# PAMRec/PAMRec

Measured on NVIDIA B200. Metric: train samples/sec, higher is better.
Workload: dtype f32

## Files before the change

### pamrec_b200/csrc/api.cu

```cuda
#include <cmath>
#include <cstdarg>
#include <cstdio>
#include <cstdlib>
#include <string>
#include <vector>

#include "comm.h"
#include "head2.h"
#include "kernels.h"
#include "layout.h"

using namespace pamrec;

struct Xchg {
  std::vector<int64_t> soff, scnt, roff, rcnt;
  int64_t n_send = 0, n_recv = 0;
};

struct PamrecHandle_ {
  PamrecConfig cfg;
  Layout L;
  PamrecBuffers buf;
  bool bound = false;
  int debug = 0;
  std::string err;
  int64_t launches = 0;
  Prof prof;
  BnSet bn[BN_COUNT];
  std::vector<int> h_seg_id, h_seg_tab;
  Comm comm;
  int* h_counts = nullptr;
  Xchg xc[3];
  bool xc_users = false;
  bool sharded() const { return cfg.table_mode == PAMREC_TABLES_SHARDED; }
  bool sibling() const { return cfg.model_kind != PAMREC_MODEL_PAMREC; }
  bool replicated() const { return cfg.table_mode == PAMREC_TABLES_REPLICATED && cfg.world_size > 1; }
  cudaStream_t side = nullptr;
  cudaEvent_t ev_side[12] = {};
  cudaEvent_t ev_join = nullptr, ev_plan = nullptr, ev_bucket = nullptr;
  int ev_next = 0;
  const void* plan_for = nullptr;
  int plan_rows = -1;
  void* mbox = nullptr;
  void* mbox_peer[kP2PMaxWorld] = {};
  bool mbox_open = false;
  unsigned* head_bar = nullptr;
  bool head_trace = false;
  unsigned long long* head_trace_cta = nullptr;
  uint32_t coop_epoch = 0;
  Head2 head2;
  int head2_grid = 0;
  bool use_head2() const { return head2_grid > 0 && (cfg.world_size == 1 || mbox_open); }
  uint32_t* mbox_err() const { return static_cast<uint32_t*>(mbox); }
  int64_t xr_dense() const { return (L.dense_numel + 63) / 64 * 64; }
  int64_t xr_floats() const { return xr_dense() + (replicated() ? sp2_rep_floats(cfg.n_items, cfg.n_cates, cfg.n_users) : 0); }
  char* xr_region(int p) const { return static_cast<char*>(mbox_peer[p]) + p2p_xr_offset(cfg.world_size); }
  bool use_xr() const { return mbox_open && cfg.world_size > 1; }
  uint32_t xr_epoch = 0;
  float* rep_grad_in() const { return use_xr() ? xr_xbuf(xr_region(cfg.rank)) + xr_dense() : wf("rep.grad"); }
  float* rep_grad_out() const {
    return use_xr() ? xr_xbuf(xr_region(cfg.rank)) + p2p_xr_cap(cfg.world_size, xr_floats()) + xr_dense() : wf("rep.grad");
  }
  ~PamrecHandle_() {
    if (h_counts) cudaFreeHost(h_counts);
    for (int p = 0; p < kP2PMaxWorld; ++p)
      if (mbox_peer[p] && mbox_peer[p] != mbox) cudaIpcCloseMemHandle(mbox_peer[p]);
    if (mbox) cudaFree(mbox);
    if (head_bar) cudaFree(head_bar);
    if (head_trace_cta) cudaFree(head_trace_cta);
    for (auto e : ev_side) if (e) cudaEventDestroy(e);
    if (ev_join) cudaEventDestroy(ev_join);
    if (ev_plan) cudaEventDestroy(ev_plan);
    if (ev_bucket) cudaEventDestroy(ev_bucket);
    if (side) cudaStreamDestroy(side);
  }
  template <typename F>
  void fork(cudaStream_t main, F fn) {
    cudaEvent_t e = ev_side[ev_next];
    ev_next = (ev_next + 1) % 12;
    cudaEventRecord(e, main);
    cudaStreamWaitEvent(side, e, 0);
    fn(side);
  }
  void join(cudaStream_t main) {
    cudaEventRecord(ev_join, side);
    cudaStreamWaitEvent(main, ev_join, 0);
  }

  float* P(int64_t off) const { return buf.dense_param + off; }
  float* G(int64_t off) const { return buf.dense_grad + off; }
  template <typename T>
  T* ws(const std::string& name) const { return reinterpret_cast<T*>(static_cast<char*>(buf.workspace) + L.ws_off(name)); }
  float* wf(const std::string& name) const { return ws<float>(name); }
  int* wi(const std::string& name) const { return ws<int>(name); }
  double* wd(const std::string& name) const { return ws<double>(name); }
};

struct ProfBind {
  PamrecHandle h; int64_t l0; Prof* prev;
  explicit ProfBind(PamrecHandle hh) : h(hh), l0(hh->prof.launches), prev(g_prof) { g_prof = &hh->prof; }
  ~ProfBind() { h->launches = h->prof.launches - l0; g_prof = prev; }
};
// ... 798 lines not shown
  const int B = b->batch, T = h->cfg.max_seq_len, N = B * T;
  int crc = 0;
  cudaMemsetAsync(h->buf.dense_grad, 0, (size_t)L.dense_numel * 4, st);
  cudaMemsetAsync(h->wd("loss_acc"), 0, 8 * sizeof(double), st);
  cudaMemsetAsync(h->wd("sp_normsq"), 0, 8 * sizeof(double), st);
  if (h->use_head2()) {
    cudaMemsetAsync(h->wd("bn.bsums"), 0, (size_t)L.ws[L.ws_index.at("bn.bsums")].numel * sizeof(double), st);
    HeadDyn d = head_dyn(h, b, true, 12);
    if (launch_head2_bwd(h->head2, d, h->head2_grid, st)) return check_cuda(h, "cooperative head launch");
    h->fork(st, [&](cudaStream_t s2) { launch_head2_dw(h->head2, B, s2); });
  } else {
    crc = head_backward(h, b, st);
  }
  float* g_a = h->wf("g_a");
  float* g_b = h->wf("g_b");
  const int max_tiles = N / kTokTile + kNB + 1;
  int* ctl = h->wi("bucket_ctl");
  for (int k = 1; k >= 0; --k) {
    const BlockOff& o = L.blk[k];
    std::string p = "blk" + std::to_string(k) + ".";
    const float* xin = k == 0 ? h->wf("x0") : h->wf("blk0.out");
    float* gout = k == 1 ? g_a : g_b;
    float* gin = k == 1 ? g_b : g_a;
    launch_ffn_bwd(h->wf(p + "y"), gout, h->P(o.w1), h->P(o.b1), h->P(o.w2), h->P(o.ln_b_beta), h->P(o.ln_b_gamma), h->wf("d_y"),
                   h->G(o.w1), h->G(o.b1), h->G(o.w2), h->G(o.b2), h->G(o.ln_b_beta), h->G(o.ln_b_gamma), N, st);
    if (T <= 128)
      launch_attn_bwd_mma(h->wf(p + "Q"), h->wf(p + "K"), h->wf(p + "V"), h->wf("d_y"), h->wf(p + "pv"), h->wf(p + "ml"),
                          b->mask, h->wf("d_Q"), h->wf("d_K"), h->wf("d_V"), B, T, st);
    else
      launch_attn_bwd(h->wf(p + "Q"), h->wf(p + "K"), h->wf(p + "V"), h->wf("d_y"), h->wf(p + "pv"), h->wf(p + "ml"),
                      b->mask, h->wf("d_Q"), h->wf("d_K"), h->wf("d_V"), B, T, st);
    launch_proj_bwd(xin, h->wf("d_y"), h->wf("d_Q"), h->wf("d_K"), h->wf("d_V"), h->wi("perm"), ctl, h->wi("tile_bucket"),
                    h->wi("tile_begin"), h->wi("tile_count"), max_tiles, h->P(o.wq), h->P(o.wk), h->P(o.wv), h->P(o.ln_a_beta),
                    h->P(o.ln_a_gamma), gin, h->G(o.wq), h->G(o.wk), h->G(o.wv), h->G(o.ln_a_beta), h->G(o.ln_a_gamma), st);
  }
  launch_embed_bwd_reduce(g_a, h->wf("d_tgt"), h->wf("d_tgt_total"), h->G(L.pos), h->wd("sp_normsq") + 4,
                          h->sharded() ? nullptr : h->wd("sp_normsq"), B, T, st);
  h->join(st);
  if (crc) return fail(h, "nccl: %s", h->comm.err.c_str());
  return check_cuda(h, "backward");
}

static void peer_allreduce_grads(PamrecHandle h, cudaStream_t st) {
  XrArgs a;
  memset(&a, 0, sizeof a);
  const int W = h->cfg.world_size;
  for (int p = 0; p < W; ++p) a.peer[p] = h->xr_region(p);
  a.world = W; a.rank = h->cfg.rank; a.epoch = ++h->xr_epoch;
  a.cap = p2p_xr_cap(W, h->xr_floats());
  a.dense_grad = h->buf.dense_grad; a.n_dense = h->L.dense_numel;
  a.scalars[0] = h->wd("sp_normsq"); a.n_scalars[0] = 8;
  a.scalars[1] = h->wd("loss_acc"); a.n_scalars[1] = 4;
  a.counter = reinterpret_cast<unsigned*>(h->xr_region(h->cfg.rank) + 128);
  a.err = h->mbox_err();
  launch_xr_allreduce(a, h->buf.dense_grad, st);
}

// ... 230 lines not shown
```

### pamrec_b200/csrc/kernels.h

```cpp
#pragma once
#include <string>
#include <vector>

#include "common.cuh"

namespace pamrec {

struct Prof {
  bool on = false;
  int64_t launches = 0;
  std::vector<std::string> names;
  std::vector<double> ms;
  std::vector<int64_t> cnt;
  struct Pair { cudaEvent_t a, b; int id; };
  std::vector<Pair> pending;
  std::vector<cudaEvent_t> free_ev;
  int id_of(const char* name);
  cudaEvent_t get_event();
  void resolve();
  void reset();
  ~Prof();
};
extern thread_local Prof* g_prof;
struct ProfScope {
  Prof* p; cudaStream_t st; cudaEvent_t b; bool timed;
  ProfScope(const char* name, int n_kernels, cudaStream_t st);
  ~ProfScope();
};
#define PAMREC_PROF(name, n, st) ProfScope _prof_scope(name, n, st)

int init_encoder_kernels(int max_T);
void launch_embed_fwd(const int* ih, const int* ch, const int* items, const int* cates, const float* item_w,
                      const float* cate_w, const float* pos, float* x0, float* tgt, int64_t n_rows, int T, cudaStream_t st);
void launch_bucket_plan(const float* lt, int n, int* bucket, int* perm, int* ctl, int* tile_bucket, int* tile_begin,
                        int* tile_count, cudaStream_t st);
void launch_proj_fwd(const float* X, const int* perm, const int* ctl, const int* tile_bucket, const int* tile_begin,
                     const int* tile_count, int max_tiles, const float* Wq, const float* Wk, const float* Wv,
                     const float* ln_beta, const float* ln_gamma, float* QIN, float* Q, float* K, float* V, cudaStream_t st);
void launch_attn_fwd(const float* Q, const float* K, const float* V, const float* QIN, const int* mask, float* Y, float* PV,
                     float* ML, int B, int T, cudaStream_t st);
void launch_ffn_fwd(const float* Y, const float* W1, const float* b1, const float* W2, const float* b2,
                    const float* ln_beta, const float* ln_gamma, float* OUT, float* Hdbg, int n_tok, cudaStream_t st);
void launch_ffn_bwd(const float* Y, const float* dOUT, const float* W1, const float* b1, const float* W2,
                    const float* ln_beta, const float* ln_gamma, float* dY, float* dW1, float* db1, float* dW2,
                    float* db2, float* dbeta, float* dgamma, int n_tok, cudaStream_t st);
void launch_attn_bwd(const float* Q, const float* K, const float* V, const float* dY, const float* PV, const float* ML,
                     const int* mask, float* dQ, float* dK, float* dV, int B, int T, cudaStream_t st);
void launch_proj_bwd(const float* X, const float* dY, const float* dQ, const float* dK, const float* dV, const int* perm,
                     const int* ctl, const int* tile_bucket, const int* tile_begin, const int* tile_count, int max_tiles,
                     const float* Wq, const float* Wk, const float* Wv, const float* ln_beta, const float* ln_gamma,
                     float* dX, float* dWq, float* dWk, float* dWv, float* dbeta, float* dgamma, cudaStream_t st);

int init_attn_mma_kernels(int max_T);
void launch_attn_fwd_mma(const float* Q, const float* K, const float* V, const float* QIN, const int* mask, float* Y, float* PV, float* ML,
                         int B, int T, cudaStream_t st);
void launch_attn_bwd_mma(const float* Q, const float* K, const float* V, const float* dY, const float* PV, const float* ML,
                         const int* mask, float* dQ, float* dK, float* dV, int B, int T, cudaStream_t st);

void launch_dense_fwd(const DenseP& p, cudaStream_t st);
void launch_dense_dx(const DenseDxP& p, cudaStream_t st);
void launch_dense_dw(const DenseDwP& p, cudaStream_t st);
void launch_bn_finalize(const BnSet& s, double count, cudaStream_t st);
void launch_bn_eval_stat(const BnSet& s, cudaStream_t st);
void launch_bn_bwd_stats(const BnSet& s, const float* dA, const float* Z, int M, cudaStream_t st);
void launch_pool_fwd(const float* H, const float* Z2, const BnSet& s1, const int* mask, float* new_long, int B, int T,
                     cudaStream_t st);
void launch_pool_bwd(const float* H, const float* Z2, const BnSet& s1, const int* mask, const float* d_new_long, float* dA2,
                     float* dH, int B, int T, cudaStream_t st);
void launch_combine_fwd(const float* ZE1, const float* ZG1, const BnSet& e1, const BnSet& g1, const float* tgt, float* U,
                        int B, cudaStream_t st);
void launch_combine_bwd(const float* ZE1, const float* ZG1, const BnSet& e1, const BnSet& g1, const float* dU, float* dE1,
                        float* dG1, float* dTgt, int B, cudaStream_t st);
void launch_loss(const float* logits, const float* y_sat, const float* y_play, const float* plays, float* d_logits,
                 double* loss_acc, int B, int B_global, const double* n_valid_global, float fuzhu_w, float order_w,
// ... 132 lines not shown
```

### pamrec_b200/csrc/kernels_encoder.cu

```cuda
#include "kernels.h"
#include "mma.cuh"

namespace pamrec {

constexpr int kEmbU = 8;
constexpr int kEmbTok = 32;
__global__ void __launch_bounds__(kEmbTok * 10, 3)
k_embed_fwd(const int* __restrict__ ih, const int* __restrict__ ch, const int* __restrict__ items,
            const int* __restrict__ cates, const float* __restrict__ item_w, const float* __restrict__ cate_w,
            const float* __restrict__ pos, float* __restrict__ x0, float* __restrict__ tgt, int64_t n_tok, int T) {
  constexpr int TOK = kEmbTok * kEmbU;
  __shared__ int s_id[4][TOK];
  __shared__ int s_t[TOK];
  const int tid = threadIdx.x;
  const int64_t tok0 = (int64_t)blockIdx.x * TOK;
  for (int i = tid; i < TOK; i += kEmbTok * 10) {
    const int64_t tok = tok0 + i;
    if (tok < n_tok) {
      const int64_t b = tok / T;
      s_t[i] = (int)(tok - b * T);
      s_id[0][i] = __ldg(ih + tok);
      s_id[1][i] = __ldg(ch + tok);
      s_id[2][i] = __ldg(items + b);
      s_id[3][i] = __ldg(cates + b);
// ... 487 lines not shown
    for (int j = 0; j < 2; ++j) {
      float a = sb[nt][j], b = sg[nt][j];
#pragma unroll
      for (int o = 4; o < 32; o <<= 1) { a += __shfl_xor_sync(0xffffffffu, a, o); b += __shfl_xor_sync(0xffffffffu, b, o); }
      if (g == 0) { atomicAdd(red + 8 * nt + 2 * t + j, a); atomicAdd(red + kD + 8 * nt + 2 * t + j, b); }
    }
}
__device__ __forceinline__ void store_frag_rows(float* __restrict__ dst, const float (&c)[kMT][5][4], int64_t tok0, const int* toks,
                                                int row_base, int cnt, int lane) {
  const int g = lane >> 2, t = lane & 3;
#pragma unroll
  for (int mt = 0; mt < kMT; ++mt)
#pragma unroll
    for (int h = 0; h < 2; ++h) {
      const int r = row_base + 16 * mt + g + 8 * h;
      if (r < cnt) {
        float* o = dst + (toks ? (int64_t)toks[r] : tok0 + r) * kD + 2 * t;
#pragma unroll
        for (int nt = 0; nt < 5; ++nt) *reinterpret_cast<float2*>(o + 8 * nt) = make_float2(c[mt][nt][2 * h], c[mt][nt][2 * h + 1]);
      }
    }
}

constexpr int kFfnBwdSmem = (4 * kDD + 3 * kTokTile * kTS + 2 * 41 * kD + 4 * kD + 2 * kD + kTokTile) * 4;
__global__ void __launch_bounds__(kTokThreads)
k_ffn_bwd(const float* __restrict__ Y, const float* __restrict__ dOUT, const float* __restrict__ W1,
          const float* __restrict__ b1, const float* __restrict__ W2, const float* __restrict__ ln_beta,
          const float* __restrict__ ln_gamma, float* __restrict__ dY, float* __restrict__ dW1, float* __restrict__ db1,
          float* __restrict__ dW2, float* __restrict__ db2, float* __restrict__ dbeta, float* __restrict__ dgamma,
          int n_tok) {
  extern __shared__ __align__(16) float sm[];
  uint32_t* W1hi = reinterpret_cast<uint32_t*>(sm);
  uint32_t* W1lo = W1hi + kDD;
  uint32_t* W2hi = W1lo + kDD;
  uint32_t* W2lo = W2hi + kDD;
  float* xs = sm + 4 * kDD;
  float* hs = xs + kTokTile * kTS;
  float* gs = hs + kTokTile * kTS;
  float* acc2 = gs + kTokTile * kTS;
  float* acc1 = acc2 + 41 * kD;
  float* pr = acc1 + 41 * kD;
  float* red = pr + 4 * kD;
  float* rstd_s = red + 2 * kD;
  const int tid = threadIdx.x, lane = tid & 31, w = tid >> 5;
  const int g = lane >> 2, t = lane & 3;
  const int64_t tok0 = (int64_t)blockIdx.x * kTokTile;
  const int cnt = (int)min((int64_t)kTokTile, (int64_t)n_tok - tok0);
  load_split_mat(W1hi, W1lo, W1, tid);
  load_split_mat(W2hi, W2lo, W2, tid);
  if (tid < kD) { pr[tid] = b1[tid]; pr[2 * kD + tid] = ln_beta[tid]; pr[3 * kD + tid] = ln_gamma[tid]; }
  if (tid < 2 * kD) red[tid] = 0.f;
  for (int i = tid; i < 2 * 41 * kD; i += kTokThreads) acc2[i] = 0.f;
  load_tile44(xs, Y + tok0 * kD, nullptr, cnt, tid);
  load_tile44(gs, dOUT + tok0 * kD, nullptr, cnt, tid);
  __syncthreads();
  if (tid < kTokTile) {
    float mean, rstd;
    ln_row44(xs + tid * kTS, pr + 2 * kD, pr + 3 * kD, mean, rstd, kLnWriteXhat);
    rstd_s[tid] = rstd;
  }
  __syncthreads();
  const float* xw = xs + kWarpRows * w * kTS;
  float* hw = hs + kWarpRows * w * kTS;
  const float* gw = gs + kWarpRows * w * kTS;
  const float* beta = pr + 2 * kD;
  const float* gamma = pr + 3 * kD;
  auto f_elem = [&](int r, int k) { return fmaf(gamma[k], xw[r * kTS + k], beta[k]); };
  float c[kMT][5][4];
#pragma unroll
  for (int mt = 0; mt < kMT; ++mt)
#pragma unroll
    for (int nt = 0; nt < 5; ++nt) {
      const float b0 = pr[8 * nt + 2 * t], bb1 = pr[8 * nt + 2 * t + 1];
      c[mt][nt][0] = b0; c[mt][nt][1] = bb1; c[mt][nt][2] = b0; c[mt][nt][3] = bb1;
    }
  warp_gemm_rows_x40x40<kMT, false>(c, f_elem, W1hi, W1lo, lane);
#pragma unroll
  for (int mt = 0; mt < kMT; ++mt)
#pragma unroll
    for (int nt = 0; nt < 5; ++nt) {
      const int r = 16 * mt + g, col = 8 * nt + 2 * t;
      *reinterpret_cast<float2*>(hw + r * kTS + col) = make_float2(fmaxf(c[mt][nt][0], 0.f), fmaxf(c[mt][nt][1], 0.f));
      *reinterpret_cast<float2*>(hw + (r + 8) * kTS + col) = make_float2(fmaxf(c[mt][nt][2], 0.f), fmaxf(c[mt][nt][3], 0.f));
    }
  __syncwarp();
#pragma unroll
  for (int mt = 0; mt < kMT; ++mt)
#pragma unroll
    for (int nt = 0; nt < 5; ++nt)
#pragma unroll
      for (int q = 0; q < 4; ++q) c[mt][nt][q] = 0.f;
  warp_gemm_rows_x40x40<kMT, true>(c, [&](int r, int k) { return gw[r * kTS + k]; }, W2hi, W2lo, lane);
#pragma unroll
  for (int mt = 0; mt < kMT; ++mt)
#pragma unroll
    for (int nt = 0; nt < 5; ++nt) {
      const int r = 16 * mt + g, col = 8 * nt + 2 * t;
      const float2 h0 = *reinterpret_cast<const float2*>(hw + r * kTS + col);
      const float2 h1 = *reinterpret_cast<const float2*>(hw + (r + 8) * kTS + col);
      if (!(h0.x > 0.f)) c[mt][nt][0] = 0.f;
      if (!(h0.y > 0.f)) c[mt][nt][1] = 0.f;
      if (!(h1.x > 0.f)) c[mt][nt][2] = 0.f;
      if (!(h1.y > 0.f)) c[mt][nt][3] = 0.f;
    }
  {
    float cw[3][5][4];
#pragma unroll
    for (int mt = 0; mt < 3; ++mt)
#pragma unroll
      for (int nt = 0; nt < 5; ++nt)
#pragma unroll
        for (int q = 0; q < 4; ++q) cw[mt][nt][q] = 0.f;
    warp_gemm_tn_48x40(cw, kWarpRows, [&](int r, int i) { return i < kD ? hw[r * kTS + i] : (i == kD ? 1.f : 0.f); },
                       [&](int r, int n) { return gw[r * kTS + n]; }, lane);
    tn_flush_smem(cw, acc2, lane);
  }
  __syncwarp();
#pragma unroll
  for (int mt = 0; mt < kMT; ++mt)
#pragma unroll
    for (int nt = 0; nt < 5; ++nt) {
      const int r = 16 * mt + g, col = 8 * nt + 2 * t;
      *reinterpret_cast<float2*>(hw + r * kTS + col) = make_float2(c[mt][nt][0], c[mt][nt][1]);
      *reinterpret_cast<float2*>(hw + (r + 8) * kTS + col) = make_float2(c[mt][nt][2], c[mt][nt][3]);
    }
  __syncwarp();
#pragma unroll
  for (int mt = 0; mt < kMT; ++mt)
#pragma unroll
    for (int nt = 0; nt < 5; ++nt) {
      const int r = 16 * mt + g, col = 8 * nt + 2 * t;
      const float2 g0 = *reinterpret_cast<const float2*>(gw + r * kTS + col);
      const float2 g1 = *reinterpret_cast<const float2*>(gw + (r + 8) * kTS + col);
      c[mt][nt][0] = g0.x; c[mt][nt][1] = g0.y; c[mt][nt][2] = g1.x; c[mt][nt][3] = g1.y;
    }
  warp_gemm_rows_x40x40<kMT, true>(c, [&](int r, int k) { return hw[r * kTS + k]; }, W1hi, W1lo, lane);
  {
    float cw[3][5][4];
#pragma unroll
    for (int mt = 0; mt < 3; ++mt)
#pragma unroll
      for (int nt = 0; nt < 5; ++nt)
#pragma unroll
        for (int q = 0; q < 4; ++q) cw[mt][nt][q] = 0.f;
    warp_gemm_tn_48x40(cw, kWarpRows, [&](int r, int i) { return i < kD ? f_elem(r, i) : (i == kD ? 1.f : 0.f); },
                       [&](int r, int n) { return hw[r * kTS + n]; }, lane);
    tn_flush_smem(cw, acc1, lane);
  }
  ln_bwd_frag(c, [&](int r, int col) { return *reinterpret_cast<const float2*>(xw + r * kTS + col); }, rstd_s + kWarpRows * w, gamma, red, lane);
  store_frag_rows(dY, c, tok0, nullptr, kWarpRows * w, cnt, lane);
  __syncthreads();
  for (int i = tid; i < kDD; i += kTokThreads) { atomicAdd(dW2 + i, acc2[i]); atomicAdd(dW1 + i, acc1[i]); }
  if (tid < kD) {
    atomicAdd(db2 + tid, acc2[kDD + tid]); atomicAdd(db1 + tid, acc1[kDD + tid]);
    atomicAdd(dbeta + tid, red[tid]); atomicAdd(dgamma + tid, red[kD + tid]);
  }
}

void launch_ffn_bwd(const float* Y, const float* dOUT, const float* W1, const float* b1, const float* W2,
                    const float* ln_beta, const float* ln_gamma, float* dY, float* dW1, float* db1, float* dW2,
                    float* db2, float* dbeta, float* dgamma, int n_tok, cudaStream_t st) {
  PAMREC_PROF("ffn_bwd", 1, st);
  if (n_tok == 0) return;
  k_ffn_bwd<<<(n_tok + kTokTile - 1) / kTokTile, kTokThreads, kFfnBwdSmem, st>>>(Y, dOUT, W1, b1, W2, ln_beta, ln_gamma, dY, dW1,
                                                                             db1, dW2, db2, dbeta, dgamma, n_tok);
}

__host__ __device__ inline int attn_bwd_per(int T) { return 4 * T * kAttnStride + ((5 * T + 4 + 3) & ~3); }
inline size_t attn_bwd_smem(int T) { return (size_t)attn_spb(T) * attn_bwd_per(T) * 4; }

__global__ void __launch_bounds__(256)
k_attn_bwd(const float* __restrict__ Q, const float* __restrict__ K, const float* __restrict__ V,
           const float* __restrict__ dY, const float* __restrict__ PV,
           const float* __restrict__ ML, const int* __restrict__ mask, float* __restrict__ dQ, float* __restrict__ dK,
           float* __restrict__ dV, int B, int T) {
  extern __shared__ __align__(16) float sm[];
  const int nw = attn_nw(T), spb = attn_spb(T), tps = nw * 32;
  const int TS = T * kAttnStride;
  const int per = attn_bwd_per(T);
  const int tid = threadIdx.x;
  const int b0 = blockIdx.x * spb;
  const int ns = min(spb, B - b0);
  for (int i = tid; i < ns * T * 10; i += blockDim.x) {
    const int sl = i / (T * 10), rc = i % (T * 10), r = rc / 10, c = rc % 10;
    const int64_t g = ((int64_t)(b0 + sl) * T + r) * kD + 4 * c;
    float* base = sm + sl * per + r * kAttnStride + 4 * c;
    st4(base, ld4(K + g));
    st4(base + TS, ld4(V + g));
// ... 64 lines not shown
    for (int tt = 0; tt < tq_end; ++tt) {
      const float* qr = Qs + tt * kAttnStride;
      const float* gr = Gs + tt * kAttnStride;
      const float sv = mkj ? dot40(kj, qr) * rscale : kMaskNeg;
      const float p = expf(sv - rm[tt]) * ril[tt];
      const float dp = dot40(vj, gr);
      const float ds = mkj ? p * (dp - rD[tt]) * rscale : 0.f;
#pragma unroll
      for (int i = 0; i < 10; ++i) { f4_fma(ak[i], ds, ld4(qr + 4 * i)); f4_fma(av[i], p, ld4(gr + 4 * i)); }
    }
#pragma unroll
    for (int i = 0; i < 10; ++i) { st4(dK + row + 4 * i, ak[i]); st4(dV + row + 4 * i, av[i]); }
  }
}

void launch_attn_bwd(const float* Q, const float* K, const float* V, const float* dY, const float* PV, const float* ML, const int* mask, float* dQ, float* dK, float* dV, int B, int T, cudaStream_t st) {
  PAMREC_PROF("attn_bwd", 1, st);
  if (B == 0) return;
  const size_t smem = attn_bwd_smem(T);
  const int spb = attn_spb(T), threads = spb * attn_nw(T) * 32;
  k_attn_bwd<<<(B + spb - 1) / spb, threads, smem, st>>>(Q, K, V, dY, PV, ML, mask, dQ, dK, dV, B, T);
}

constexpr int kProjBwdSmem = (6 * kDD + 2 * kTokTile * kTS + kDD + 2 * kD + 2 * kD + 2 * kTokTile) * 4;
__global__ void __launch_bounds__(kTokThreads)
k_proj_bwd(const float* __restrict__ X, const float* __restrict__ dY, const float* __restrict__ dQ,
           const float* __restrict__ dK, const float* __restrict__ dV, const int* __restrict__ perm,
           const int* __restrict__ ctl, const int* __restrict__ tile_bucket, const int* __restrict__ tile_begin,
           const int* __restrict__ tile_count, const float* __restrict__ Wq, const float* __restrict__ Wk,
           const float* __restrict__ Wv, const float* __restrict__ ln_beta, const float* __restrict__ ln_gamma,
           float* __restrict__ dX, float* __restrict__ dWq, float* __restrict__ dWk, float* __restrict__ dWv,
           float* __restrict__ dbeta, float* __restrict__ dgamma) {
  int tile = blockIdx.x;
  if (tile >= ctl[32]) return;
  extern __shared__ __align__(16) float sm[];
  uint32_t* Whi = reinterpret_cast<uint32_t*>(sm);
  uint32_t* Wlo = Whi + 3 * kDD;
  float* xs = sm + 6 * kDD;
  float* gs = xs + kTokTile * kTS;
  float* acc = gs + kTokTile * kTS;
  float* lnp = acc + kDD;
  float* red = lnp + 2 * kD;
  float* mean_s = red + 2 * kD;
  float* rstd_s = mean_s + kTokTile;
  __shared__ int toks[kTokTile];
  const int tid = threadIdx.x, lane = tid & 31, w = tid >> 5;
  const int g = lane >> 2, t = lane & 3;
  const int k = tile_bucket[tile], begin = tile_begin[tile], cnt = tile_count[tile];
  const bool zero = k == kZeroBin;
  load_split_mat(Whi, Wlo, zero ? nullptr : Wq + (int64_t)k * kDD, tid);
  load_split_mat(Whi + kDD, Wlo + kDD, zero ? nullptr : Wk + (int64_t)k * kDD, tid);
  load_split_mat(Whi + 2 * kDD, Wlo + 2 * kDD, zero ? nullptr : Wv + (int64_t)k * kDD, tid);
  if (tid < kD) { lnp[tid] = ln_beta[tid]; lnp[kD + tid] = ln_gamma[tid]; }
  if (tid < 2 * kD) red[tid] = 0.f;
  for (int i = tid; i < kDD; i += kTokThreads) acc[i] = 0.f;
  if (tid < cnt) toks[tid] = perm[begin + tid];
  __syncthreads();
  load_tile44(xs, X, toks, cnt, tid);
  load_tile44(gs, dQ, toks, cnt, tid);
  __syncthreads();
  if (tid < kTokTile) {
    float mean, rstd;
    ln_row44(xs + tid * kTS, lnp, lnp + kD, mean, rstd, 0);
    mean_s[tid] = mean; rstd_s[tid] = rstd;
  }
  __syncthreads();
  const float* xw = xs + kWarpRows * w * kTS;
  const float* gw = gs + kWarpRows * w * kTS;
  const float* mw = mean_s + kWarpRows * w;
  const float* rw = rstd_s + kWarpRows * w;
  const float* beta = lnp;
  const float* gamma = lnp + kD;
  auto xhat = [&](int r, int i) { return (xw[r * kTS + i] - mw[r]) * rw[r]; };
  auto g_elem = [&](int r, int kk) { return gw[r * kTS + kk]; };
  float dqin[kMT][5][4], dx[kMT][5][4];
#pragma unroll
  for (int mt = 0; mt < kMT; ++mt)
#pragma unroll
    for (int h = 0; h < 2; ++h) {
      const int r = kWarpRows * w + 16 * mt + g + 8 * h;
      const float* src = dY + (int64_t)toks[r < cnt ? r : 0] * kD + 2 * t;
#pragma unroll
      for (int nt = 0; nt < 5; ++nt) {
        const float2 v = r < cnt ? *reinterpret_cast<const float2*>(src + 8 * nt) : make_float2(0.f, 0.f);
        dqin[mt][nt][2 * h] = v.x; dqin[mt][nt][2 * h + 1] = v.y;
      }
    }
  warp_gemm_rows_x40x40<kMT, true>(dqin, g_elem, Whi, Wlo, lane);
  {
    float cw[3][5][4];
#pragma unroll
    for (int mt = 0; mt < 3; ++mt)
#pragma unroll
      for (int nt = 0; nt < 5; ++nt)
#pragma unroll
        for (int q = 0; q < 4; ++q) cw[mt][nt][q] = 0.f;
    warp_gemm_tn_48x40(cw, kWarpRows, [&](int r, int i) { return i < kD ? fmaf(gamma[i], xhat(r, i), beta[i]) : 0.f; }, g_elem, lane);
    tn_flush_smem(cw, acc, lane, kD - 1);
  }
  float* dWs[3] = {dWq + (int64_t)k * kDD, dWk + (int64_t)k * kDD, dWv + (int64_t)k * kDD};
  auto flush_acc = [&](float* dW) {
    __syncthreads();
    for (int i = tid; i < kDD; i += kTokThreads) { if (!zero) atomicAdd(dW + i, acc[i]); acc[i] = 0.f; }
  };
  flush_acc(dWs[0]);
#pragma unroll
  for (int mt = 0; mt < kMT; ++mt)
#pragma unroll
    for (int nt = 0; nt < 5; ++nt)
#pragma unroll
      for (int q = 0; q < 4; ++q) dx[mt][nt][q] = 0.f;
#pragma unroll 1
  for (int m = 1; m < 3; ++m) {
    __syncthreads();
    load_tile44(gs, m == 1 ? dK : dV, toks, cnt, tid);
    __syncthreads();
    warp_gemm_rows_x40x40<kMT, true>(dx, g_elem, Whi + m * kDD, Wlo + m * kDD, lane);
    float cw[3][5][4];
#pragma unroll
    for (int mt = 0; mt < 3; ++mt)
#pragma unroll
      for (int nt = 0; nt < 5; ++nt)
#pragma unroll
        for (int q = 0; q < 4; ++q) cw[mt][nt][q] = 0.f;
    warp_gemm_tn_48x40(cw, kWarpRows, [&](int r, int i) { return i < kD ? xw[r * kTS + i] : 0.f; }, g_elem, lane);
    tn_flush_smem(cw, acc, lane, kD - 1);
    flush_acc(dWs[m]);
  }
  ln_bwd_frag(dqin, [&](int r, int col) { return make_float2(xhat(r, col), xhat(r, col + 1)); }, rw, gamma, red, lane);
#pragma unroll
  for (int mt = 0; mt < kMT; ++mt)
#pragma unroll
    for (int nt = 0; nt < 5; ++nt)
#pragma unroll
      for (int q = 0; q < 4; ++q) dx[mt][nt][q] += dqin[mt][nt][q];
  store_frag_rows(dX, dx, 0, toks, kWarpRows * w, cnt, lane);
  __syncthreads();
  if (tid < kD) { atomicAdd(dbeta + tid, red[tid]); atomicAdd(dgamma + tid, red[kD + tid]); }
}

void launch_proj_bwd(const float* X, const float* dY, const float* dQ, const float* dK, const float* dV, const int* perm,
                     const int* ctl, const int* tile_bucket, const int* tile_begin, const int* tile_count, int max_tiles,
                     const float* Wq, const float* Wk, const float* Wv, const float* ln_beta, const float* ln_gamma,
                     float* dX, float* dWq, float* dWk, float* dWv, float* dbeta, float* dgamma, cudaStream_t st) {
  PAMREC_PROF("proj_bwd", 1, st);
  k_proj_bwd<<<max_tiles, kTokThreads, kProjBwdSmem, st>>>(X, dY, dQ, dK, dV, perm, ctl, tile_bucket, tile_begin, tile_count, Wq,
                                                        Wk, Wv, ln_beta, ln_gamma, dX, dWq, dWk, dWv, dbeta, dgamma);
}

int init_encoder_kernels(int max_T) {
  cudaError_t e = cudaSuccess;
  auto set = [&](const void* fn, size_t bytes) {
    if (e == cudaSuccess) e = cudaFuncSetAttribute(fn, cudaFuncAttributeMaxDynamicSharedMemorySize, (int)bytes);
  };
  set((const void*)k_proj_fwd, kProjFwdSmem);
  set((const void*)k_ffn_fwd, kFfnFwdSmem);
  set((const void*)k_ffn_bwd, kFfnBwdSmem);
  set((const void*)k_proj_bwd, kProjBwdSmem);
  size_t af = 0, ab = 0;
  for (int T = 1; T <= max_T; ++T) { af = af > attn_fwd_smem(T) ? af : attn_fwd_smem(T); ab = ab > attn_bwd_smem(T) ? ab : attn_bwd_smem(T); }
  set((const void*)k_attn_fwd, af);
  set((const void*)k_attn_bwd, ab);
  return e == cudaSuccess ? 0 : -1;
}

}
```

### pamrec_b200/csrc/layout.h

```cpp
#pragma once
#include <cstdio>
#include <cstring>
#include <map>
#include <string>
#include <vector>

#include "common.cuh"

namespace pamrec {

struct TensorDesc {
  std::string name;
  int pool = 0, dtype = PAMREC_F32, flags = 0;
  int64_t offset = 0, numel = 0;
  int ndim = 0;
  int64_t shape[4] = {0, 0, 0, 0};
};

struct BlockOff { int64_t ln_a_beta, ln_a_gamma, wq, wk, wv, w1, b1, w2, b2, ln_b_beta, ln_b_gamma; };
struct MlpOff { int64_t w0, b0, g0, be0, w1, b1, g1, be1, wout, bout; };
struct BnOff { int C; int64_t gamma, beta, mm, mv; };

enum BnId { BN_S0 = 0, BN_S1, BN_E0, BN_G0, BN_E1, BN_G1, BN_T0, BN_T1, BN_COUNT };

// ... 355 lines not shown
    add_ws("zt1", PAMREC_F32, {B, 192});
    add_ws("logits", PAMREC_F32, {B, 3});
    add_ws("losses", PAMREC_F32, {8});
    add_ws("loss_acc", PAMREC_F64, {8});
    add_ws("d_logits", PAMREC_F32, {B, 3});
    add_ws("d_t1", PAMREC_F32, {B, 192});
    add_ws("d_t0", PAMREC_F32, {B, 300});
    add_ws("d_u", PAMREC_F32, {B, 168});
    add_ws("d_e1", PAMREC_F32, {B, 320});
    add_ws("d_g1", PAMREC_F32, {B, 10});
    add_ws("d_e0", PAMREC_F32, {B, 500});
    add_ws("d_g0", PAMREC_F32, {B, 128});
    add_ws("d_new_long", PAMREC_F32, {B, kD});
    add_ws("d_tgt", PAMREC_F32, {B, kE});
    add_ws("d_tgt_total", PAMREC_F32, {B, kE});
    add_ws("d_z2", PAMREC_F32, {B, T});
    add_ws("d_a1", PAMREC_F32, {B, T, 20});
    add_ws("g_a", PAMREC_F32, {B, T, kD});
    add_ws("g_b", PAMREC_F32, {B, T, kD});
    add_ws("d_y", PAMREC_F32, {B, T, kD});
    add_ws("d_Q", PAMREC_F32, {B, T, kD});
    add_ws("d_K", PAMREC_F32, {B, T, kD});
    add_ws("d_V", PAMREC_F32, {B, T, kD});
    add_bn_ws();
    add_optim_ws();
    const int64_t NK = N + B;
    const bool sharded = table_mode == PAMREC_TABLES_SHARDED;
    cub_keys_table = NK;
    for (const char* t : {"item", "cate"}) {
      std::string p = std::string("sp.") + t + ".";
      if (sharded) {
        add_ws(p + "keys", PAMREC_I32, {NK});
        add_ws(p + "idx", PAMREC_I32, {NK});
        add_ws(p + "skeys", PAMREC_I32, {NK});
        add_ws(p + "sidx", PAMREC_I32, {NK});
        add_ws(p + "uidx", PAMREC_I32, {NK});
        add_ws(p + "slot", PAMREC_I32, {rows_of(t[0] == 'i' ? n_items : n_cates)});
      }
      add_ws(p + "ukeys", PAMREC_I32, {NK});
      add_ws(p + "accum", PAMREC_F32, {NK, t[0] == 'i' ? kI : kC});
    }
    if (sharded) {
      add_ws("sp.user.keys", PAMREC_I32, {B});
      add_ws("sp.user.idx", PAMREC_I32, {B});
      add_ws("sp.user.skeys", PAMREC_I32, {B});
      add_ws("sp.user.sidx", PAMREC_I32, {B});
// ... 53 lines not shown
```

Measured before the change: 1.336 million.

## Split encoder weight-gradient GEMMs into separate kernel overlapped on side stream

Removes the per-tile weight-gradient accumulation (dW1/dW2/db, dWq/dWk/dWv) from the FFN and projection backward kernels. Those kernels now spill the hidden activation, masked dH, and (for block 1) dOUT to new workspace buffers. A new k_enc_dw kernel recomputes the weight gradients from these buffers with a cp.async double-buffered GEMM over token runs and runs on the side stream, overlapping with attention and projection backward. This shortens the critical-path kernels, lowers their shared memory use and per-tile atomics, and cuts global atomic traffic. In exchange it adds extra global writes and reads of activations, new workspace buffers, and duplicated dQ/dK/dV storage for block 1 so the overlap stays safe.

```diff
diff --git a/pamrec_b200/csrc/api.cu b/pamrec_b200/csrc/api.cu
--- a/pamrec_b200/csrc/api.cu
+++ b/pamrec_b200/csrc/api.cu
@@ -36,7 +36,7 @@
   bool sibling() const { return cfg.model_kind != PAMREC_MODEL_PAMREC; }
   bool replicated() const { return cfg.table_mode == PAMREC_TABLES_REPLICATED && cfg.world_size > 1; }
   cudaStream_t side = nullptr;
-  cudaEvent_t ev_side[12] = {};
+  cudaEvent_t ev_side[16] = {};
   cudaEvent_t ev_join = nullptr, ev_plan = nullptr, ev_bucket = nullptr;
   int ev_next = 0;
   const void* plan_for = nullptr;
@@ -77,7 +77,7 @@
   template <typename F>
   void fork(cudaStream_t main, F fn) {
     cudaEvent_t e = ev_side[ev_next];
-    ev_next = (ev_next + 1) % 12;
+    ev_next = (ev_next + 1) % 16;
     cudaEventRecord(e, main);
     cudaStreamWaitEvent(side, e, 0);
     fn(side);
@@ -922,17 +922,27 @@
     const float* xin = k == 0 ? h->wf("x0") : h->wf("blk0.out");
     float* gout = k == 1 ? g_a : g_b;
     float* gin = k == 1 ? g_b : g_a;
+    float* dQ = h->wf(k == 1 ? "blk1.d_Q" : "d_Q");
+    float* dK = h->wf(k == 1 ? "blk1.d_K" : "d_K");
+    float* dV = h->wf(k == 1 ? "blk1.d_V" : "d_V");
+    float* dout = k == 1 ? h->wf("blk1.d_out") : gout;
+    EncDwArgs dw{h->wf(p + "qin"), xin, dQ, dK, dV, h->wi("perm"), ctl, h->wf(p + "y"), h->P(o.ln_b_beta), h->P(o.ln_b_gamma),
+                 h->wf(p + "h"), h->wf(p + "dhr"), dout, h->G(o.wq), h->G(o.wk), h->G(o.wv), h->G(o.w1), h->G(o.b1), h->G(o.w2),
+                 h->G(o.b2), N, true};
     launch_ffn_bwd(h->wf(p + "y"), gout, h->P(o.w1), h->P(o.b1), h->P(o.w2), h->P(o.ln_b_beta), h->P(o.ln_b_gamma), h->wf("d_y"),
-                   h->G(o.w1), h->G(o.b1), h->G(o.w2), h->G(o.b2), h->G(o.ln_b_beta), h->G(o.ln_b_gamma), N, st);
+                   h->wf(p + "h"), h->wf(p + "dhr"), k == 1 ? dout : nullptr, h->G(o.ln_b_beta), h->G(o.ln_b_gamma), N, st);
+    h->fork(st, [&](cudaStream_t s2) { launch_enc_dw(dw, s2); });
     if (T <= 128)
       launch_attn_bwd_mma(h->wf(p + "Q"), h->wf(p + "K"), h->wf(p + "V"), h->wf("d_y"), h->wf(p + "pv"), h->wf(p + "ml"),
-                          b->mask, h->wf("d_Q"), h->wf("d_K"), h->wf("d_V"), B, T, st);
+                          b->mask, dQ, dK, dV, B, T, st);
     else
       launch_attn_bwd(h->wf(p + "Q"), h->wf(p + "K"), h->wf(p + "V"), h->wf("d_y"), h->wf(p + "pv"), h->wf(p + "ml"),
-                      b->mask, h->wf("d_Q"), h->wf("d_K"), h->wf("d_V"), B, T, st);
-    launch_proj_bwd(xin, h->wf("d_y"), h->wf("d_Q"), h->wf("d_K"), h->wf("d_V"), h->wi("perm"), ctl, h->wi("tile_bucket"),
-                    h->wi("tile_begin"), h->wi("tile_count"), max_tiles, h->P(o.wq), h->P(o.wk), h->P(o.wv), h->P(o.ln_a_beta),
-                    h->P(o.ln_a_gamma), gin, h->G(o.wq), h->G(o.wk), h->G(o.wv), h->G(o.ln_a_beta), h->G(o.ln_a_gamma), st);
+                      b->mask, dQ, dK, dV, B, T, st);
+    dw.ffn = false;
+    h->fork(st, [&](cudaStream_t s2) { launch_enc_dw(dw, s2); });
+    launch_proj_bwd(xin, h->wf("d_y"), dQ, dK, dV, h->wi("perm"), ctl, h->wi("tile_bucket"), h->wi("tile_begin"), h->wi("tile_count"),
+                    max_tiles, h->P(o.wq), h->P(o.wk), h->P(o.wv), h->P(o.ln_a_beta), h->P(o.ln_a_gamma), gin, h->G(o.ln_a_beta),
+                    h->G(o.ln_a_gamma), st);
   }
   launch_embed_bwd_reduce(g_a, h->wf("d_tgt"), h->wf("d_tgt_total"), h->G(L.pos), h->wd("sp_normsq") + 4,
                           h->sharded() ? nullptr : h->wd("sp_normsq"), B, T, st);
diff --git a/pamrec_b200/csrc/kernels.h b/pamrec_b200/csrc/kernels.h
--- a/pamrec_b200/csrc/kernels.h
+++ b/pamrec_b200/csrc/kernels.h
@@ -42,14 +42,25 @@
 void launch_ffn_fwd(const float* Y, const float* W1, const float* b1, const float* W2, const float* b2,
                     const float* ln_beta, const float* ln_gamma, float* OUT, float* Hdbg, int n_tok, cudaStream_t st);
 void launch_ffn_bwd(const float* Y, const float* dOUT, const float* W1, const float* b1, const float* W2,
-                    const float* ln_beta, const float* ln_gamma, float* dY, float* dW1, float* db1, float* dW2,
-                    float* db2, float* dbeta, float* dgamma, int n_tok, cudaStream_t st);
+                    const float* ln_beta, const float* ln_gamma, float* dY, float* H, float* DHR, float* dOUT_keep,
+                    float* dbeta, float* dgamma, int n_tok, cudaStream_t st);
 void launch_attn_bwd(const float* Q, const float* K, const float* V, const float* dY, const float* PV, const float* ML,
                      const int* mask, float* dQ, float* dK, float* dV, int B, int T, cudaStream_t st);
 void launch_proj_bwd(const float* X, const float* dY, const float* dQ, const float* dK, const float* dV, const int* perm,
                      const int* ctl, const int* tile_bucket, const int* tile_begin, const int* tile_count, int max_tiles,
                      const float* Wq, const float* Wk, const float* Wv, const float* ln_beta, const float* ln_gamma,
-                     float* dX, float* dWq, float* dWk, float* dWv, float* dbeta, float* dgamma, cudaStream_t st);
+                     float* dX, float* dbeta, float* dgamma, cudaStream_t st);
+struct EncDwArgs {
+  const float* qin; const float* x; const float* dQ; const float* dK; const float* dV;
+  const int* perm; const int* ctl;
+  const float* y; const float* ln_beta; const float* ln_gamma;
+  const float* h; const float* dhr; const float* dout;
+  float* dWq; float* dWk; float* dWv;
+  float* dW1; float* db1; float* dW2; float* db2;
+  int n_tok;
+  bool ffn;
+};
+void launch_enc_dw(const EncDwArgs& a, cudaStream_t st);
 
 int init_attn_mma_kernels(int max_T);
 void launch_attn_fwd_mma(const float* Q, const float* K, const float* V, const float* QIN, const int* mask, float* Y, float* PV, float* ML,
diff --git a/pamrec_b200/csrc/kernels_encoder.cu b/pamrec_b200/csrc/kernels_encoder.cu
--- a/pamrec_b200/csrc/kernels_encoder.cu
+++ b/pamrec_b200/csrc/kernels_encoder.cu
@@ -533,13 +533,12 @@
     }
 }
 
-constexpr int kFfnBwdSmem = (4 * kDD + 3 * kTokTile * kTS + 2 * 41 * kD + 4 * kD + 2 * kD + kTokTile) * 4;
+constexpr int kFfnBwdSmem = (4 * kDD + 3 * kTokTile * kTS + 4 * kD + 2 * kD + kTokTile) * 4;
 __global__ void __launch_bounds__(kTokThreads)
 k_ffn_bwd(const float* __restrict__ Y, const float* __restrict__ dOUT, const float* __restrict__ W1,
           const float* __restrict__ b1, const float* __restrict__ W2, const float* __restrict__ ln_beta,
-          const float* __restrict__ ln_gamma, float* __restrict__ dY, float* __restrict__ dW1, float* __restrict__ db1,
-          float* __restrict__ dW2, float* __restrict__ db2, float* __restrict__ dbeta, float* __restrict__ dgamma,
-          int n_tok) {
+          const float* __restrict__ ln_gamma, float* __restrict__ dY, float* __restrict__ H, float* __restrict__ DHR,
+          float* __restrict__ DOUT_KEEP, float* __restrict__ dbeta, float* __restrict__ dgamma, int n_tok) {
   extern __shared__ __align__(16) float sm[];
   uint32_t* W1hi = reinterpret_cast<uint32_t*>(sm);
   uint32_t* W1lo = W1hi + kDD;
@@ -548,9 +547,7 @@
   float* xs = sm + 4 * kDD;
   float* hs = xs + kTokTile * kTS;
   float* gs = hs + kTokTile * kTS;
-  float* acc2 = gs + kTokTile * kTS;
-  float* acc1 = acc2 + 41 * kD;
-  float* pr = acc1 + 41 * kD;
+  float* pr = gs + kTokTile * kTS;
   float* red = pr + 4 * kD;
   float* rstd_s = red + 2 * kD;
   const int tid = threadIdx.x, lane = tid & 31, w = tid >> 5;
@@ -561,7 +558,6 @@
   load_split_mat(W2hi, W2lo, W2, tid);
   if (tid < kD) { pr[tid] = b1[tid]; pr[2 * kD + tid] = ln_beta[tid]; pr[3 * kD + tid] = ln_gamma[tid]; }
   if (tid < 2 * kD) red[tid] = 0.f;
-  for (int i = tid; i < 2 * 41 * kD; i += kTokThreads) acc2[i] = 0.f;
   load_tile44(xs, Y + tok0 * kD, nullptr, cnt, tid);
   load_tile44(gs, dOUT + tok0 * kD, nullptr, cnt, tid);
   __syncthreads();
@@ -570,6 +566,8 @@
     ln_row44(xs + tid * kTS, pr + 2 * kD, pr + 3 * kD, mean, rstd, kLnWriteXhat);
     rstd_s[tid] = rstd;
   }
+  if (DOUT_KEEP != nullptr)
+    for (int i = tid; i < cnt * 10; i += kTokThreads) st4(DOUT_KEEP + (tok0 + i / 10) * kD + 4 * (i % 10), ld4(gs + (i / 10) * kTS + 4 * (i % 10)));
   __syncthreads();
   const float* xw = xs + kWarpRows * w * kTS;
   float* hw = hs + kWarpRows * w * kTS;
@@ -591,9 +589,12 @@
 #pragma unroll
     for (int nt = 0; nt < 5; ++nt) {
       const int r = 16 * mt + g, col = 8 * nt + 2 * t;
-      *reinterpret_cast<float2*>(hw + r * kTS + col) = make_float2(fmaxf(c[mt][nt][0], 0.f), fmaxf(c[mt][nt][1], 0.f));
-      *reinterpret_cast<float2*>(hw + (r + 8) * kTS + col) = make_float2(fmaxf(c[mt][nt][2], 0.f), fmaxf(c[mt][nt][3], 0.f));
-    }
+#pragma unroll
+      for (int q = 0; q < 4; ++q) c[mt][nt][q] = fmaxf(c[mt][nt][q], 0.f);
+      *reinterpret_cast<float2*>(hw + r * kTS + col) = make_float2(c[mt][nt][0], c[mt][nt][1]);
+      *reinterpret_cast<float2*>(hw + (r + 8) * kTS + col) = make_float2(c[mt][nt][2], c[mt][nt][3]);
+    }
+  store_frag_rows(H, c, tok0, nullptr, kWarpRows * w, cnt, lane);
   __syncwarp();
 #pragma unroll
   for (int mt = 0; mt < kMT; ++mt)
@@ -614,18 +615,7 @@
       if (!(h1.x > 0.f)) c[mt][nt][2] = 0.f;
       if (!(h1.y > 0.f)) c[mt][nt][3] = 0.f;
     }
-  {
-    float cw[3][5][4];
-#pragma unroll
-    for (int mt = 0; mt < 3; ++mt)
-#pragma unroll
-      for (int nt = 0; nt < 5; ++nt)
-#pragma unroll
-        for (int q = 0; q < 4; ++q) cw[mt][nt][q] = 0.f;
-    warp_gemm_tn_48x40(cw, kWarpRows, [&](int r, int i) { return i < kD ? hw[r * kTS + i] : (i == kD ? 1.f : 0.f); },
-                       [&](int r, int n) { return gw[r * kTS + n]; }, lane);
-    tn_flush_smem(cw, acc2, lane);
-  }
+  store_frag_rows(DHR, c, tok0, nullptr, kWarpRows * w, cnt, lane);
   __syncwarp();
 #pragma unroll
   for (int mt = 0; mt < kMT; ++mt)
@@ -646,35 +636,19 @@
       c[mt][nt][0] = g0.x; c[mt][nt][1] = g0.y; c[mt][nt][2] = g1.x; c[mt][nt][3] = g1.y;
     }
   warp_gemm_rows_x40x40<kMT, true>(c, [&](int r, int k) { return hw[r * kTS + k]; }, W1hi, W1lo, lane);
-  {
-    float cw[3][5][4];
-#pragma unroll
-    for (int mt = 0; mt < 3; ++mt)
-#pragma unroll
-      for (int nt = 0; nt < 5; ++nt)
-#pragma unroll
-        for (int q = 0; q < 4; ++q) cw[mt][nt][q] = 0.f;
-    warp_gemm_tn_48x40(cw, kWarpRows, [&](int r, int i) { return i < kD ? f_elem(r, i) : (i == kD ? 1.f : 0.f); },
-                       [&](int r, int n) { return hw[r * kTS + n]; }, lane);
-    tn_flush_smem(cw, acc1, lane);
-  }
   ln_bwd_frag(c, [&](int r, int col) { return *reinterpret_cast<const float2*>(xw + r * kTS + col); }, rstd_s + kWarpRows * w, gamma, red, lane);
   store_frag_rows(dY, c, tok0, nullptr, kWarpRows * w, cnt, lane);
   __syncthreads();
-  for (int i = tid; i < kDD; i += kTokThreads) { atomicAdd(dW2 + i, acc2[i]); atomicAdd(dW1 + i, acc1[i]); }
-  if (tid < kD) {
-    atomicAdd(db2 + tid, acc2[kDD + tid]); atomicAdd(db1 + tid, acc1[kDD + tid]);
-    atomicAdd(dbeta + tid, red[tid]); atomicAdd(dgamma + tid, red[kD + tid]);
-  }
+  if (tid < kD) { atomicAdd(dbeta + tid, red[tid]); atomicAdd(dgamma + tid, red[kD + tid]); }
 }
 
 void launch_ffn_bwd(const float* Y, const float* dOUT, const float* W1, const float* b1, const float* W2,
-                    const float* ln_beta, const float* ln_gamma, float* dY, float* dW1, float* db1, float* dW2,
-                    float* db2, float* dbeta, float* dgamma, int n_tok, cudaStream_t st) {
+                    const float* ln_beta, const float* ln_gamma, float* dY, float* H, float* DHR, float* dOUT_keep,
+                    float* dbeta, float* dgamma, int n_tok, cudaStream_t st) {
   PAMREC_PROF("ffn_bwd", 1, st);
   if (n_tok == 0) return;
-  k_ffn_bwd<<<(n_tok + kTokTile - 1) / kTokTile, kTokThreads, kFfnBwdSmem, st>>>(Y, dOUT, W1, b1, W2, ln_beta, ln_gamma, dY, dW1,
-                                                                             db1, dW2, db2, dbeta, dgamma, n_tok);
+  k_ffn_bwd<<<(n_tok + kTokTile - 1) / kTokTile, kTokThreads, kFfnBwdSmem, st>>>(Y, dOUT, W1, b1, W2, ln_beta, ln_gamma, dY, H, DHR,
+                                                                             dOUT_keep, dbeta, dgamma, n_tok);
 }
 
 __host__ __device__ inline int attn_bwd_per(int T) { return 4 * T * kAttnStride + ((5 * T + 4 + 3) & ~3); }
@@ -785,15 +759,14 @@
   k_attn_bwd<<<(B + spb - 1) / spb, threads, smem, st>>>(Q, K, V, dY, PV, ML, mask, dQ, dK, dV, B, T);
 }
 
-constexpr int kProjBwdSmem = (6 * kDD + 2 * kTokTile * kTS + kDD + 2 * kD + 2 * kD + 2 * kTokTile) * 4;
+constexpr int kProjBwdSmem = (6 * kDD + 2 * kTokTile * kTS + 2 * kD + 2 * kD + 2 * kTokTile) * 4;
 __global__ void __launch_bounds__(kTokThreads)
 k_proj_bwd(const float* __restrict__ X, const float* __restrict__ dY, const float* __restrict__ dQ,
            const float* __restrict__ dK, const float* __restrict__ dV, const int* __restrict__ perm,
            const int* __restrict__ ctl, const int* __restrict__ tile_bucket, const int* __restrict__ tile_begin,
            const int* __restrict__ tile_count, const float* __restrict__ Wq, const float* __restrict__ Wk,
            const float* __restrict__ Wv, const float* __restrict__ ln_beta, const float* __restrict__ ln_gamma,
-           float* __restrict__ dX, float* __restrict__ dWq, float* __restrict__ dWk, float* __restrict__ dWv,
-           float* __restrict__ dbeta, float* __restrict__ dgamma) {
+           float* __restrict__ dX, float* __restrict__ dbeta, float* __restrict__ dgamma) {
   int tile = blockIdx.x;
   if (tile >= ctl[32]) return;
   extern __shared__ __align__(16) float sm[];
@@ -801,8 +774,7 @@
   uint32_t* Wlo = Whi + 3 * kDD;
   float* xs = sm + 6 * kDD;
   float* gs = xs + kTokTile * kTS;
-  float* acc = gs + kTokTile * kTS;
-  float* lnp = acc + kDD;
+  float* lnp = gs + kTokTile * kTS;
   float* red = lnp + 2 * kD;
   float* mean_s = red + 2 * kD;
   float* rstd_s = mean_s + kTokTile;
@@ -816,7 +788,6 @@
   load_split_mat(Whi + 2 * kDD, Wlo + 2 * kDD, zero ? nullptr : Wv + (int64_t)k * kDD, tid);
   if (tid < kD) { lnp[tid] = ln_beta[tid]; lnp[kD + tid] = ln_gamma[tid]; }
   if (tid < 2 * kD) red[tid] = 0.f;
-  for (int i = tid; i < kDD; i += kTokThreads) acc[i] = 0.f;
   if (tid < cnt) toks[tid] = perm[begin + tid];
   __syncthreads();
   load_tile44(xs, X, toks, cnt, tid);
@@ -832,7 +803,6 @@
   const float* gw = gs + kWarpRows * w * kTS;
   const float* mw = mean_s + kWarpRows * w;
   const float* rw = rstd_s + kWarpRows * w;
-  const float* beta = lnp;
   const float* gamma = lnp + kD;
   auto xhat = [&](int r, int i) { return (xw[r * kTS + i] - mw[r]) * rw[r]; };
   auto g_elem = [&](int r, int kk) { return gw[r * kTS + kk]; };
@@ -850,23 +820,6 @@
       }
     }
   warp_gemm_rows_x40x40<kMT, true>(dqin, g_elem, Whi, Wlo, lane);
-  {
-    float cw[3][5][4];
-#pragma unroll
-    for (int mt = 0; mt < 3; ++mt)
-#pragma unroll
-      for (int nt = 0; nt < 5; ++nt)
-#pragma unroll
-        for (int q = 0; q < 4; ++q) cw[mt][nt][q] = 0.f;
-    warp_gemm_tn_48x40(cw, kWarpRows, [&](int r, int i) { return i < kD ? fmaf(gamma[i], xhat(r, i), beta[i]) : 0.f; }, g_elem, lane);
-    tn_flush_smem(cw, acc, lane, kD - 1);
-  }
-  float* dWs[3] = {dWq + (int64_t)k * kDD, dWk + (int64_t)k * kDD, dWv + (int64_t)k * kDD};
-  auto flush_acc = [&](float* dW) {
-    __syncthreads();
-    for (int i = tid; i < kDD; i += kTokThreads) { if (!zero) atomicAdd(dW + i, acc[i]); acc[i] = 0.f; }
-  };
-  flush_acc(dWs[0]);
 #pragma unroll
   for (int mt = 0; mt < kMT; ++mt)
 #pragma unroll
@@ -879,16 +832,6 @@
     load_tile44(gs, m == 1 ? dK : dV, toks, cnt, tid);
     __syncthreads();
     warp_gemm_rows_x40x40<kMT, true>(dx, g_elem, Whi + m * kDD, Wlo + m * kDD, lane);
-    float cw[3][5][4];
-#pragma unroll
-    for (int mt = 0; mt < 3; ++mt)
-#pragma unroll
-      for (int nt = 0; nt < 5; ++nt)
-#pragma unroll
-        for (int q = 0; q < 4; ++q) cw[mt][nt][q] = 0.f;
-    warp_gemm_tn_48x40(cw, kWarpRows, [&](int r, int i) { return i < kD ? xw[r * kTS + i] : 0.f; }, g_elem, lane);
-    tn_flush_smem(cw, acc, lane, kD - 1);
-    flush_acc(dWs[m]);
   }
   ln_bwd_frag(dqin, [&](int r, int col) { return make_float2(xhat(r, col), xhat(r, col + 1)); }, rw, gamma, red, lane);
 #pragma unroll
@@ -905,10 +848,107 @@
 void launch_proj_bwd(const float* X, const float* dY, const float* dQ, const float* dK, const float* dV, const int* perm,
                      const int* ctl, const int* tile_bucket, const int* tile_begin, const int* tile_count, int max_tiles,
                      const float* Wq, const float* Wk, const float* Wv, const float* ln_beta, const float* ln_gamma,
-                     float* dX, float* dWq, float* dWk, float* dWv, float* dbeta, float* dgamma, cudaStream_t st) {
+                     float* dX, float* dbeta, float* dgamma, cudaStream_t st) {
   PAMREC_PROF("proj_bwd", 1, st);
   k_proj_bwd<<<max_tiles, kTokThreads, kProjBwdSmem, st>>>(X, dY, dQ, dK, dV, perm, ctl, tile_bucket, tile_begin, tile_count, Wq,
-                                                        Wk, Wv, ln_beta, ln_gamma, dX, dWq, dWk, dWv, dbeta, dgamma);
+                                                        Wk, Wv, ln_beta, ln_gamma, dX, dbeta, dgamma);
+}
+
+constexpr int kDwRun = 256;
+constexpr int kEncDwSmem = (4 * kTokTile * kTS + 41 * kD + 2 * kD) * 4;
+__device__ __forceinline__ void cp_async16(float* dst, const float* src, bool valid) {
+  const unsigned d = (unsigned)__cvta_generic_to_shared(dst);
+  asm volatile("cp.async.cg.shared.global [%0], [%1], 16, %2;\n" ::"r"(d), "l"(src), "r"(valid ? 16 : 0));
+}
+__global__ void __launch_bounds__(kTokThreads)
+k_enc_dw(const EncDwArgs a) {
+  extern __shared__ __align__(16) float sm[];
+  float* acc = sm + 4 * kTokTile * kTS;
+  float* lnp = acc + 41 * kD;
+  __shared__ int s_cnt[kNB];
+  const int tid = threadIdx.x, lane = tid & 31, w = tid >> 5;
+  if (tid < kD) { lnp[tid] = a.ln_beta[tid]; lnp[kD + tid] = a.ln_gamma[tid]; }
+  if (tid < kNB) s_cnt[tid] = a.ctl[tid];
+  __syncthreads();
+  const int s_lo = a.ffn ? 0 : 2, s_hi = a.ffn ? 2 : 2 + 3 * kNB;
+  int64_t total = 0;
+  if (a.ffn) total = 2 * (int64_t)a.n_tok;
+  else for (int k = 0; k < kNB; ++k) total += 3 * (int64_t)s_cnt[k];
+  const int64_t chunk = (total + gridDim.x - 1) / gridDim.x;
+  const int64_t lo = blockIdx.x * chunk, hi = min(total, lo + chunk);
+  const int lr = tid >> 1, c0 = 5 * (tid & 1);
+  int64_t v = 0;
+  int bin0 = 0;
+  for (int s = s_lo; s < s_hi && v < hi; ++s) {
+    const int k = s < 2 ? -1 : (s - 2) / 3, p = s < 2 ? -1 : (s - 2) % 3;
+    const int64_t len = s < 2 ? a.n_tok : s_cnt[k];
+    const int64_t b = max(lo, v) - v, e = min(hi, v + len) - v;
+    v += len;
+    if (b < e) {
+      const bool bias = s < 2;
+      const float* A = s == 0 ? a.y : s == 1 ? a.h : p == 0 ? a.qin : a.x;
+      const float* Bm = s == 0 ? a.dhr : s == 1 ? a.dout : p == 0 ? a.dQ : p == 1 ? a.dK : a.dV;
+      const int* rows = bias ? nullptr : a.perm + bin0;
+      float* dW = s == 0 ? a.dW1 : s == 1 ? a.dW2 : (p == 0 ? a.dWq : p == 1 ? a.dWk : a.dWv) + (int64_t)k * kDD;
+      float* db = s == 0 ? a.db1 : a.db2;
+      for (int i = tid; i < 41 * kD; i += kTokThreads) acc[i] = 0.f;
+      float cw[3][5][4];
+#pragma unroll
+      for (int mt = 0; mt < 3; ++mt)
+#pragma unroll
+        for (int nt = 0; nt < 5; ++nt)
+#pragma unroll
+          for (int q = 0; q < 4; ++q) cw[mt][nt][q] = 0.f;
+      auto row_of = [&](int64_t i) -> int64_t { return i < e ? (rows ? (int64_t)rows[i] : i) : -1; };
+      auto issue = [&](int buf, int64_t r) {
+        float* da = sm + 2 * buf * kTokTile * kTS + lr * kTS + 4 * c0;
+        const int64_t o = (r >= 0 ? r : 0) * kD + 4 * c0;
+#pragma unroll
+        for (int j = 0; j < 5; ++j) {
+          cp_async16(da + 4 * j, A + o + 4 * j, r >= 0);
+          cp_async16(da + kTokTile * kTS + 4 * j, Bm + o + 4 * j, r >= 0);
+        }
+        asm volatile("cp.async.commit_group;\n" ::);
+      };
+      issue(0, row_of(b + lr));
+      int64_t nxt = row_of(b + kTokTile + lr);
+      int buf = 0;
+      for (int64_t t0 = b; t0 < e; t0 += kTokTile, buf ^= 1) {
+        if (t0 + kTokTile < e) issue(buf ^ 1, nxt);
+        else asm volatile("cp.async.commit_group;\n" ::);
+        nxt = row_of(t0 + 2 * kTokTile + lr);
+        asm volatile("cp.async.wait_group 1;\n" ::);
+        __syncthreads();
+        float* As = sm + 2 * buf * kTokTile * kTS;
+        if (s == 0) {
+          if (tid < kTokTile) { float mean, rstd; ln_row44(As + tid * kTS, lnp, lnp + kD, mean, rstd, kLnWriteF); }
+          __syncthreads();
+        }
+        const float* aw = As + kWarpRows * w * kTS;
+        const float* bw = aw + kTokTile * kTS;
+        warp_gemm_tn_48x40(cw, kWarpRows, [&](int r, int i) { return i < kD ? aw[r * kTS + i] : (i == kD && bias ? 1.f : 0.f); },
+                           [&](int r, int n) { return bw[r * kTS + n]; }, lane);
+        __syncthreads();
+      }
+      tn_flush_smem(cw, acc, lane, bias ? kD : kD - 1);
+      __syncthreads();
+      for (int i = tid; i < kDD; i += kTokThreads) atomicAdd(dW + i, acc[i]);
+      if (bias && tid < kD) atomicAdd(db + tid, acc[kDD + tid]);
+      __syncthreads();
+    }
+    if (p == 2) bin0 += s_cnt[k];
+  }
+}
+
+void launch_enc_dw(const EncDwArgs& a, cudaStream_t st) {
+  PAMREC_PROF("enc_dw", 1, st);
+  if (a.n_tok == 0) return;
+  int dev = 0, n_sm = 0;
+  cudaGetDevice(&dev);
+  cudaDeviceGetAttribute(&n_sm, cudaDevAttrMultiProcessorCount, dev);
+  const int64_t runs = ((a.ffn ? 2 : 3) * (int64_t)a.n_tok + kDwRun - 1) / kDwRun;
+  const int grid = (int)(runs < 2 * n_sm ? runs : 2 * n_sm);
+  k_enc_dw<<<grid, kTokThreads, kEncDwSmem, st>>>(a);
 }
 
 int init_encoder_kernels(int max_T) {
@@ -920,6 +960,7 @@
   set((const void*)k_ffn_fwd, kFfnFwdSmem);
   set((const void*)k_ffn_bwd, kFfnBwdSmem);
   set((const void*)k_proj_bwd, kProjBwdSmem);
+  set((const void*)k_enc_dw, kEncDwSmem);
   size_t af = 0, ab = 0;
   for (int T = 1; T <= max_T; ++T) { af = af > attn_fwd_smem(T) ? af : attn_fwd_smem(T); ab = ab > attn_bwd_smem(T) ? ab : attn_bwd_smem(T); }
   set((const void*)k_attn_fwd, af);
diff --git a/pamrec_b200/csrc/layout.h b/pamrec_b200/csrc/layout.h
--- a/pamrec_b200/csrc/layout.h
+++ b/pamrec_b200/csrc/layout.h
@@ -401,6 +401,8 @@
     add_ws("d_Q", PAMREC_F32, {B, T, kD});
     add_ws("d_K", PAMREC_F32, {B, T, kD});
     add_ws("d_V", PAMREC_F32, {B, T, kD});
+    for (const char* n : {"blk1.d_Q", "blk1.d_K", "blk1.d_V", "blk1.d_out"}) add_ws(n, PAMREC_F32, {B, T, kD});
+    for (const char* n : {"blk0.h", "blk0.dhr", "blk1.h", "blk1.dhr"}) add_ws(n, PAMREC_F32, {B, T, kD});
     add_bn_ws();
     add_optim_ws();
     const int64_t NK = N + B;
```

Result: faster. 1.383 million (median of 6 runs) (+3.5%).
